# ViennaRNA/RNAcode

Measured on AMD Instinct MI355X. Metric: alignment-columns x samples scored /sec, higher is better.
Workload: dtype f32; 1 GPU; synthetic MAF 10000 blocks x 120 cols x 6 seqs, n=1000 (BASELINE configs[2]/[3]); exchange=none, fit_exp_mode=fused

## Files before the change

rnacode_amd/csrc/rc_context.cpp:

```cpp
#include <cstddef>

#include "rc_runtime.h"

extern "C" {

const char *rc_last_error(void) { return g_err.c_str(); }

void rc_default_params(rc_params *p) {
  p->Delta = -10.0f; p->Omega = -4.0f; p->omega = -2.0f;
  p->stopPenalty_0 = -9999.0f; p->stopPenalty_k = -8.0f;
  p->blosum = 62; p->sampleN = 100; p->cutoff = 1.0f; p->stopEarly = 0; p->seed_base = 42;
  std::memset(p->genetic_code, 0, sizeof p->genetic_code);
}

}

void want_hw_queues() { (void)setenv("GPU_MAX_HW_QUEUES", "8", 0); }

int table_set(rc_ctx *c, const rc_params &par, const TableSet **out) {
  char code[64];
  const char *why = nullptr;
  if (!parse_genetic_code(par.genetic_code, code, &why)) return fail(RC_ERR_ARG, why);
  if (par.blosum != 62 && par.blosum != 90) return fail(RC_ERR_ARG, "blosum must be 62 or 90");
  std::lock_guard<std::mutex> lk(c->setMutex);
  for (const auto &t : c->sets)
    if (t->blosum == par.blosum && std::memcmp(t->code, code, 64) == 0) { *out = t.get(); return RC_OK; }
  auto t = std::make_unique<TableSet>(code, par.blosum);
  t->pt.build(t->ct);
  const size_t oPair = 0, oBlosum = al256(4096), oInfo = oBlosum + al256(400 * sizeof(int)), oPep = oInfo + al256(64 * sizeof(CodeInfo)),
               oOff = oPep + al256(64 * sizeof(int)), oAb = oOff + al256(6 * sizeof(int)), total = oAb + al256(4096 * sizeof(uint16_t));
  std::vector<uint8_t> h(total, 0);
  std::memcpy(h.data() + oPair, t->pt.pair, 4096);
  int *bl = reinterpret_cast<int *>(h.data() + oBlosum);
  for (int p = 0; p < 20; p++) for (int q = 0; q < 20; q++) bl[20 * p + q] = t->ct.blosum[p][q];
  std::memcpy(h.data() + oInfo, t->pt.info, 64 * sizeof(CodeInfo));
  int *pep = reinterpret_cast<int *>(h.data() + oPep);
  for (int i = 0; i < 64; i++) pep[i] = t->ct.pep[i];
  int *off = reinterpret_cast<int *>(h.data() + oOff);
  uint16_t *ab = reinterpret_cast<uint16_t *>(h.data() + oAb);
  int n = 0;
  off[0] = 0;
  for (int a = 0; a < 64; a++) for (int b = 0; b < 64; b++) if (pep[a] == -1 || pep[b] == -1) ab[n++] = static_cast<uint16_t>(a << 6 | b);
  for (int hq = 0; hq < 4; hq++) {
    off[1 + hq] = n;
    for (int a = 0; a < 64; a++) for (int b = 0; b < 64; b++) {
      if (pep[a] == -1 || pep[b] == -1) continue;
      const int x = a ^ b;
      if (((x & 48) != 0) + ((x & 12) != 0) + ((x & 3) != 0) == hq) ab[n++] = static_cast<uint16_t>(a << 6 | b);
    }
  }
  off[5] = n;
  t->d.retired = c->retired.get();
  HIP_TRY(hipSetDevice(c->device));
  HIP_TRY(t->d.ensure(total));
  HIP_TRY(hipMemcpy(t->d.p, h.data(), total, hipMemcpyHostToDevice));
  const uint8_t *d = t->d.as<uint8_t>();
  const CodeTables standard(par.blosum);
  t->ptrs = TablePtrs{d + oPair, reinterpret_cast<const int *>(d + oPep), reinterpret_cast<const int *>(d + oBlosum),
                      reinterpret_cast<const CodeInfo *>(d + oInfo), reinterpret_cast<const int *>(d + oOff),
                      reinterpret_cast<const uint16_t *>(d + oAb), std::memcmp(standard.pep, t->ct.pep, sizeof standard.pep) == 0};
  *out = t.get();
  c->sets.push_back(std::move(t));
  return RC_OK;
}

extern "C" {

int rc_device_count(void) {
  want_hw_queues();
  int n = 0;
  if (hipGetDeviceCount(&n) != hipSuccess) return 0;
  return n;
}

int rc_host_cpus(void) { return effective_cpus(); }

void rc_ctx_trim(rc_ctx *c) {
  if (!c) return;
  (void)hipSetDevice(c->device);
  (void)hipDeviceSynchronize();
  c->retired->drain();
  c->bufPool->drain(false);
}

void rc_ctx_destroy(rc_ctx *c) {
  if (!c) return;
  (void)hipSetDevice(c->device);
  (void)hipDeviceSynchronize();
  c->retired->ctxGone.store(true);
  c->retired->drain();
  g_retired.drain();
  c->bufPool->drain(true);
  c->pool.reset();
  if (kProfiling && c->d_cellStats.p) {
    unsigned long long st[6] = {0, 0, 0, 0, 0, 0};
    if (hipMemcpy(st, c->d_cellStats.p, sizeof st, hipMemcpyDeviceToHost) == hipSuccess && st[0])
      std::fprintf(stderr, "[rc cell stats] wavefront-cells %llu, with no positive lane %llu (%.4f %%), positive lane-cells %.2f %%\n", st[0], st[1],
                   100.0 * st[1] / st[0], 100.0 * st[2] / (64.0 * st[0])),
      std::fprintf(stderr, "[rc cell stats] before the row's first event %.1f %%, event codons %.1f %%, after its last event %.1f %%, between events %.1f %%\n",
                   100.0 * st[3] / st[0], 100.0 * st[4] / st[0], 100.0 * st[5] / st[0], 100.0 * (st[0] - st[3] - st[4] - st[5]) / st[0]);
  }
  if (c->d_U) (void)hipFree(c->d_U);
  for (hipStream_t st : c->compute) if (st) (void)hipStreamDestroy(st);
  if (c->native) (void)hipStreamDestroy(c->native);
  if (c->copy) (void)hipStreamDestroy(c->copy);
  if (c->aux) (void)hipStreamDestroy(c->aux);
  if (c->tree) (void)hipStreamDestroy(c->tree);
  if (c->tree2) (void)hipStreamDestroy(c->tree2);
  for (hipStream_t st : c->classStreams) (void)hipStreamDestroy(st);
  delete c;
}

int rc_ctx_create(int device, rc_ctx **out) {
  if (!out) return fail(RC_ERR_ARG, "null out pointer");
  *out = nullptr;
  want_hw_queues();
  int n = 0;
  trace("ctx: start", nullptr);
  if (hipGetDeviceCount(&n) != hipSuccess || n <= 0)
    return fail(RC_ERR_DEVICE, "no HIP device available: the scoring path has no CPU fallback");
  trace("ctx: runtime up", nullptr);
  if (device < 0 || device >= n) return fail(RC_ERR_ARG, "device index out of range");
  HIP_TRY(hipSetDevice(device));
  std::unique_ptr<rc_ctx, void (*)(rc_ctx *)> guard(new rc_ctx(), rc_ctx_destroy);
  rc_ctx *c = guard.get();
  c->device = device;
  hipDeviceProp_t prop;
  HIP_TRY(hipGetDeviceProperties(&prop, device));
  c->numCU = prop.multiProcessorCount;
  c->totalMem = prop.totalGlobalMem;
  c->retiredCapBytes = prop.totalGlobalMem / 16;
  c->bufPool->devCap = prop.totalGlobalMem / 16;
  c->bufPool->device = device;
  static const int hostExp = exp_mode_of_host();
  c->expMode = hostExp;
  if (const char *e = std::getenv("RC_FIT_EXP")) {
    const std::string v(e);
    if (v == "generic" || v == "1") c->expMode = 1;
    else if (v == "fused" || v == "fma" || v == "2") c->expMode = 2;
    else if (v == "device" || v == "0") c->expMode = 0;
    else return fail(RC_ERR_ARG, "RC_FIT_EXP must be generic, fused or device");
  }
  for (DevBuf *d : {&c->treeJobs, &c->treeIn, &c->treeWork, &c->treeRes, &c->d_cellStats}) d->retired = c->retired.get();
  for (PinBuf *h : {&c->treeInPin, &c->treeResPin}) h->retired = c->retired.get();
  c->genericScratchWords = std::max<size_t>(static_cast<size_t>(1) << 30, prop.totalGlobalMem / 12 / sizeof(uint32_t));
  c->togetherWords = std::max<size_t>(static_cast<size_t>(1) << 30, prop.totalGlobalMem / 36 / sizeof(uint32_t));
  if (const char *e = std::getenv("RC_TOGETHER_MAX_MB")) c->togetherWords = static_cast<size_t>(std::max(0ll, std::atoll(e))) * (1u << 20) / sizeof(uint32_t);
  if (const char *e = std::getenv("RC_CLASS_STREAMS")) c->classStreamCount = std::max(1, std::min(16, std::atoi(e)));
  if (const char *e = std::getenv("RC_GRID_CAP_PER_CU")) c->gridCapPerCU = std::max(0, std::atoi(e));
  if (const char *e = std::getenv("RC_SPLIT_FACTOR")) c->splitFactor = std::max(0.0, std::atof(e));
  if (const char *e = std::getenv("RC_NATIVE_WAVES_PER_CU")) c->nativeWavesPerCU = std::max(1, std::min(32, std::atoi(e)));
  if (const char *e = std::getenv("RC_TAIL_SHARING")) c->tailSharing = std::atoi(e) != 0;
  if (const char *e = std::getenv("RC_ROW_SPLIT")) c->rowSplit = std::atoi(e) != 0;
  if (const char *e = std::getenv("RC_HIGH_OCCUPANCY")) c->highOccupancy = std::max(0, std::min(2, std::atoi(e)));
  if (prop.maxSharedMemoryPerMultiProcessor > 0) c->ldsPerCU = prop.maxSharedMemoryPerMultiProcessor;
  if (const char *e = std::getenv("RC_FAT_STREAM_MIN_ITEMS")) c->fatStreamMinItems = std::max(0ll, std::atoll(e));
  if (const char *e = std::getenv("RC_GENERIC_SCRATCH_MB")) c->genericScratchWords = std::max<size_t>(1, static_cast<size_t>(std::atoll(e))) * (1u << 20) / sizeof(uint32_t);
  int prioLow = 0, prioHigh = 0;
  HIP_TRY(hipDeviceGetStreamPriorityRange(&prioLow, &prioHigh));
  c->prioLow = prioLow; c->prioHigh = 0; c->classPrio = prioLow;
  trace("ctx: streams", nullptr);
  c->serialNative = std::getenv("RC_SERIAL_NATIVE") ? 1 : 0;
  c->stopTwoRoundsMinItems = 4LL * c->numCU * 16;
  if (const char *e = std::getenv("RC_STOP_MIN_ITEMS")) c->stopTwoRoundsMinItems = std::atoll(e);
  if (const char *e = std::getenv("RC_GENERIC_MIN_ROWS")) c->rule.genericMinRows = std::max(3, std::min(kTemplRows + 1, std::atoi(e)));
  if (const char *e = std::getenv("RC_TILED_MAX_L")) c->rule.tiledMaxL = std::max(0, std::atoi(e));
  if (const char *e = std::getenv("RC_TILED_MIN_ROWS")) c->rule.tiledMinRows = std::max(kTiledMaxKT + 2, std::min(kTemplRows + 1, std::atoi(e)));
  if (const char *e = std::getenv("RC_TILED_MAX_ROWS")) c->rule.tiledMaxRows = std::max(kTemplRows, std::min(kMaxRows, std::atoi(e)));
  if (const char *e = std::getenv("RC_TILED_WIDE_MAX_L")) c->rule.tiledWideMaxL = std::max(0, std::atoi(e));
  if (const char *e = std::getenv("RC_TILED_ANY_L_MIN_ROWS")) c->rule.tiledAnyLMinRows = std::max(kTemplRows + 1, std::atoi(e));
  if (const char *e = std::getenv("RC_STOP_ROUNDS")) c->stopRounds = std::max(2, std::min(kMaxRounds, std::atoi(e)));
  {
    rc_params std{};
    std.blosum = 62;
    const TableSet *unused = nullptr;
    RC_TRY(table_set(c, std, &unused));
    std.blosum = 90;
    RC_TRY(table_set(c, std, &unused));
  }
  trace("ctx: tables", nullptr);
  c->tieThr = float_threshold_lt(0.0001);
  if (const char *e = std::getenv("RC_LDS_MAX_BYTES")) { c->ldsMaxBytes = c->ldsMaxBytesOneRow = static_cast<size_t>(std::atol(e)); c->stageManyRows = true; }
#ifdef RC_PROFILING
  if (const char *e = std::getenv("RC_DEBUG_SKIP")) c->debugSkip = std::atoi(e);
  if (std::getenv("RC_CELL_STATS")) {
    HIP_TRY(c->d_cellStats.ensure(6 * sizeof(unsigned long long)));
    HIP_TRY(hipMemset(c->d_cellStats.p, 0, 6 * sizeof(unsigned long long)));
  }
#endif
  c->hostThreads = std::min(effective_cpus(), 32);
  if (const char *e = std::getenv("RC_HOST_THREADS")) c->hostThreads = std::max(1, std::atoi(e));
  *out = guard.release();
  return RC_OK;
}

int rc_genetic_code(int32_t ncbi_id, char out[65]) {
  if (!out) return fail(RC_ERR_ARG, "null out pointer");
  const char *aas = ncbi_code(ncbi_id);
  if (!aas) return fail(RC_ERR_ARG, "unknown genetic code id " + std::to_string(ncbi_id) +
                                    " (built in: 1-6, 9-14, 16, 21-26, 29, 30, 33; 27, 28, 31 and 32 are not supported)");
  std::memcpy(out, aas, 64);
  out[64] = '\0';
  return RC_OK;
}

int rc_ctx_set_host_threads(rc_ctx *c, int32_t threads) {
  if (!c || threads < 1) return fail(RC_ERR_ARG, "bad argument");
  if (c->inflight.load() != 0) return fail(RC_ERR_ARG, "batches are in flight");
  c->hostThreads = threads;
  c->pool.reset();
  return RC_OK;
}

int rc_ctx_host_threads(const rc_ctx *c) { return c ? c->hostThreads : 0; }

int rc_ctx_fit_exp_mode(const rc_ctx *c) { return c ? c->expMode : RC_ERR_ARG; }

}

#undef rc_default_params
#undef rc_batch_create
#undef rc_stream_create
static constexpr size_t kParamsV1Bytes = offsetof(rc_params, genetic_code);
static_assert(kParamsV1Bytes == 40, "the members of the older rc_params layout");
static rc_params params_v1(const rc_params *old) {
  rc_params p;
  std::memset(&p, 0, sizeof p);
  std::memcpy(&p, old, kParamsV1Bytes);
  return p;
}

extern "C" {

void rc_default_params(rc_params *p) {
  rc_params q;
  rc_default_params_v2(&q);
  std::memcpy(p, &q, kParamsV1Bytes);
}

int rc_batch_create(rc_ctx *ctx, const rc_block *blocks, int32_t n_blocks, const rc_params *par, rc_batch **out) {
  if (!par) return rc_batch_create_v2(ctx, blocks, n_blocks, par, out);
  const rc_params p = params_v1(par);
  return rc_batch_create_v2(ctx, blocks, n_blocks, &p, out);
}

int rc_stream_create(rc_ctx *ctx, const rc_params *par, int32_t depth, rc_stream **out) {
  if (!par) return rc_stream_create_v2(ctx, par, depth, out);
  const rc_params p = params_v1(par);
  return rc_stream_create_v2(ctx, &p, depth, out);
}

}
```

rnacode_amd/csrc/rc_launch.h:

```cpp
#pragma once
#include <hip/hip_runtime.h>

#include <cstddef>
#include <cstdint>
#include <string>

#include "rc_device.h"

namespace rc {

#ifdef RC_PROFILING
constexpr bool kProfiling = true;
#else
constexpr bool kProfiling = false;
#endif

struct NullArgs {
  const uint8_t *blob;
  const DevBlock *dblocks;
  const int *classBlocks;
  int nClassBlocks;
  const int *nBlocksPtr;
  const uint32_t *flags;
  uint32_t skipMask;
  uint32_t onlyMask;
  int tiledKT;
  int gLo, gHi;
  int sampleN;
  int Spad;
  const uint32_t *U;
  const uint8_t *pair;
  uint32_t *scratch;
  size_t scratchStride;
  float *maxima;
  unsigned long long *clampCount;
  float tieThr;
  int comboSplit;
  unsigned int *workCounter;
  unsigned int *steal;
  uint8_t *codesAll;
  size_t codesStride;
  int cacheSites;
  int reserved[3];
  int stealWait;
  int simParts, simGrid;
  unsigned int *simCounter;
  int rowParts;
  float *sbuf;
  size_t sbufStride;
  int debugSkip;
  unsigned long long *cellStats;
};

struct NativeArgs {
  uint8_t *blob;
  const DevBlock *dblocks;
  const int *blocks;
  const uint8_t *pair;
  float *tile;
  size_t tileStride;
  int nItems;
  float *fullS;
  float *sAll;
  int sAllSites;
  DevHss *hss;
  int *hssCount;
  int hssCap;
  float tieThr;
  const uint32_t *flags;
};

struct PrepArgs {
  uint8_t *blob;
  const DevBlock *dblocks;
  const int *blocks;
  int nBlocks;
  const int *modelPrefix;
  int nModels;
  const int *pep;
  bool standardCode;
  const int *prepOff;
  const uint16_t *prepAb;
  const int *blosum;
  const CodeInfo *codeInfo;
  uint32_t *flags;
  int *exactList;
  int *exactCount;
  int classOff[kClassSlots];
  ClassRule rule;
};

struct FitOut {
  double mu, lambda;
  int rc;
  int better;
};

struct FitArgs {
// ... 178 lines not shown
```

rnacode_amd/csrc/rc_null_kernel.h:

```cpp
#pragma once
#include <hip/hip_runtime.h>

#include <type_traits>
#include <utility>

#include "rc_device.h"
#include "rc_launch.h"
#include "rc_sim_core.h"

namespace rc {


template <bool SEM> __device__ __forceinline__ float ref_max(float x, float y) {
  if constexpr (SEM) return x > y ? x : y;
  else return fmaxf(x, y);
}
template <bool SEM> __device__ __forceinline__ float ref_max3(float x, float y, float z) { return ref_max<SEM>(ref_max<SEM>(x, y), z); }

template <bool SEM = false>
__device__ __forceinline__ void pair_step(int zc, float sig, float Delta, float Omega, float omega,
                                          float &s0, float &s1, float &s2) {
  if (zc == 0) {
    s0 = s0 + sig;
    s1 = s1 + omega;
// ... 423 lines not shown
            static_for<QB>([&](auto xc) {
              constexpr int x = decltype(xc)::value;
              wait_draws(ubq[x], std::integral_constant<int, SPI * (QB - 1 - x)>{});
              if (q0 + x < nnodes) node_step(q0 + x, ubq[x], [] {});
            });
          }
        } else {
          for (int q = 0; q < nnodes; q++) {
            uint32_t u[SPI];
            if constexpr (!kLean) {
#pragma unroll
              for (int t = 0; t < SPI; t++) u[t] = Ustream[ubase[t] + q * qstride];
              node_step_plain(q, u);
              continue;
            }
            fetch_draws(u, ub[0], ub[1], ub[2], ub[3]);
#pragma unroll
            for (int t = 0; t < SPI; t++) ub[t] += qstrideB;
            node_step(q, u, [&] { wait_draws(u, std::integral_constant<int, 0>{}); });
          }
        }
#pragma unroll
        for (int t = 0; t < SPI; t++) {
          const int i = i0 + t;
          if (i <= L) {
#pragma unroll
            for (int r = 0; r < N; r++) {
              const uint32_t tip = get_state(ns[t], static_cast<int>((qtipw[r >> 2] >> (8 * (r & 3))) & 255u));
              win[r] = sim_window(win[r], tip);
              if constexpr (kRevWindow) winR[r] = sim_window_rev(winR[r], tip);
            }
            if (i >= 3 && (!SIM || (i >= iLo && i <= iHi))) {
              const int ip = L + 3 - i;
              const uint32_t aF = win[0] & 63u;
              uint32_t aR = kRevWindow ? sim_rev_codon(winR[0]) : sim_ref_rev(aF);
              asm("" : "+v"(aR));
              uint8_t *siteF = reinterpret_cast<uint8_t *>(cod + static_cast<size_t>(0 * L1 + i) * PSW);
              uint8_t *siteR = reinterpret_cast<uint8_t *>(cod + static_cast<size_t>(1 * L1 + ip) * PSW);
#pragma unroll
              for (int w = 0; w < NCW; w++) {
                uint32_t wf = 0, wr = 0;
                const uint32_t mF = maskw[(0 * L1 + i) * NCW + w], mR = maskw[(1 * L1 + ip) * NCW + w];
#pragma unroll
                for (int c = 0; c < CPW; c++) {
                  const int k = w * CPW + c;
                  if (k < NK) {
                    wf |= sim_pack(pairLut[sim_index_fwd(aF, win[k + 1], sim_mask_field(mF, c))], c);
                    if constexpr (kRevWindow) wr |= sim_pack(pairLut[sim_index_rev_window(aR, winR[k + 1], sim_mask_field(mR, c))], c);
                    else wr |= sim_pack(pairLut[sim_index_rev(aR, win[k + 1], sim_mask_field(mR, c))], c);
                  }
                }
                if (w < NCW - 1) {
                  store_words(std::integral_constant<int, 4>{}, laneWord, wf, wr, siteF + w * kWave * 4, siteR + w * kWave * 4);
                } else {
                  store_words(std::integral_constant<int, LB>{}, laneTailB, wf, wr, siteF + (NCW - 1) * kWave * 4, siteR + (NCW - 1) * kWave * 4);
                }
              }
            }
          }
        }
      }
      if (clamped && (kLean ? lane == 0 : sidx < A.sampleN) && (SIM || onlyCombo <= 0)) atomicAdd(A.clampCount, static_cast<unsigned long long>(clamped));
    }
    if constexpr (SIM) continue;
    if (!helping && shared) {
      const size_t G = gridDim.x;
      if (lane == 0) {
        __hip_atomic_store(A.steal + kStealHdr + G + 2 * blockIdx.x, static_cast<unsigned int>(bi), __ATOMIC_RELAXED, __HIP_MEMORY_SCOPE_AGENT);
        __hip_atomic_store(A.steal + kStealHdr + G + 2 * blockIdx.x + 1, static_cast<unsigned int>(grp), __ATOMIC_RELAXED, __HIP_MEMORY_SCOPE_AGENT);
      }
      __builtin_amdgcn_fence(__ATOMIC_RELEASE, "agent");
      __builtin_amdgcn_s_waitcnt(0);
      if (lane == 0) {
        atomicExch(A.steal + kStealHdr + blockIdx.x, 1u);
        const unsigned int idx = atomicAdd(A.steal, 1u);
        __hip_atomic_store(A.steal + kStealHdr + 3 * G + idx, (blockIdx.x + 1u) | (static_cast<unsigned int>(home) << 24), __ATOMIC_RELAXED, __HIP_MEMORY_SCOPE_AGENT);
        atomicSub(A.steal + 1, 1u);
      }
      firstCombo = claim_part(slot);
    }

    float best = -1.0f;
    unsigned long long statCells = 0, statNoPos = 0, statPosLanes = 0, statPristine = 0, statEvent = 0, statTail = 0;
    float omega_v, Delta_v = 0.0f;
    asm volatile("v_mov_b32 %0, %1" : "=v"(omega_v) : "s"(omega));
    float rcpNk_v = 0.0f, negNk_v = 0.0f;
    if constexpr (!EXACT && (NK & (NK - 1)) != 0) {
      asm volatile("v_mov_b32 %0, %1" : "=v"(rcpNk_v) : "s"(1.0f / static_cast<float>(NK)));
      asm volatile("v_mov_b32 %0, %1" : "=v"(negNk_v) : "s"(-static_cast<float>(NK)));
    }
    if constexpr (EXACT) asm volatile("v_mov_b32 %0, %1" : "=v"(Delta_v) : "s"(Delta));
    if (!kProfiling || !(A.debugSkip & 1)) {
      Regs R;
      int curS = -1;
      for (int c = onlyCombo >= 0 ? onlyCombo : firstCombo; c < 6; c = onlyCombo >= 0 ? 6 : (shared ? claim_part(slot) : c + 1)) {
        const int s = c >= 3 ? 1 : 0, f = c - 3 * s;
        if (s != curS) {
          static_for<NK>([&](auto kc) {
            constexpr int k = decltype(kc)::value;
            R.template at<k>().lut = __float_as_int(lut[(s * NK + k) * kLutSize + lane]);
            if constexpr (kTableLookups) lds_codes[k * kWave + lane] = static_cast<uint32_t>(R.template at<k>().lut);
          });
          curS = s;
        }
        const int sites = (L - f) / 3;
        if (sites <= 0) continue;
        const uint32_t *__restrict__ sbase = cod + static_cast<size_t>(s * L1 + 3 + f) * PSW;
        constexpr int kSiteWords = 3 * PSW;
        auto word_at = [&](int j, int x) -> uint32_t {
          const uint32_t *p = sbase + static_cast<size_t>(j) * kSiteWords;
          if (x < NCW - 1) return p[x * kWave + lane];
          return static_cast<uint32_t>(reinterpret_cast<const TailT *>(p + (NCW - 1) * kWave)[lane]);
        };
        const unsigned long long *__restrict__ zbase = zw + static_cast<size_t>(s * L1 + 3 + f) * ZW;
        const unsigned long long *__restrict__ zany = zmask + static_cast<size_t>(s * 3 + f) * zmWords;
        int jc = sites;
        constexpr int kCacheSiteBytes = PSW * 4;
        if constexpr (LDSC) {
          for (int idx = 0; idx < sites * NCW; idx++) lds_codes[idx * kWave + lane] = word_at(idx / NCW, idx % NCW);
          __builtin_amdgcn_s_waitcnt(0);
        } else if constexpr (!EXACT) {
          jc = sites - (A.cacheSites < sites ? A.cacheSites : sites);
          for (int j = jc; j < sites; j++) {
            uint32_t *dst = lds_codes + kTableWords + (j - jc) * PSW;
#pragma unroll
            for (int x = 0; x < NCW - 1; x++) dst[x * kWave + lane] = word_at(j, x);
            reinterpret_cast<TailT *>(dst + (NCW - 1) * kWave)[lane] = static_cast<TailT>(word_at(j, NCW - 1));
          }
          __builtin_amdgcn_s_waitcnt(0);
        }
        const uint32_t ldsBase = static_cast<uint32_t>(reinterpret_cast<uintptr_t>(lds_codes + kTableWords));
        const uint32_t ldsLane = ldsBase + static_cast<uint32_t>(lane) * 4u;
        const uint32_t ldsTail = ldsBase + (NCW - 1) * kWave * 4u + static_cast<uint32_t>(lane) * LB;
        const uint32_t laneOff = static_cast<uint32_t>(lane) * 4u, laneTail = static_cast<uint32_t>(lane) * LB;
        [[maybe_unused]] const uint8_t *ldsBytesAll = reinterpret_cast<const uint8_t *>(lds_codes + kTableWords) - ldsBase;
        auto fetch_staged = [&](uint32_t (&w)[NCW], int j) {
          const uint32_t at = ldsLane + static_cast<uint32_t>(j) * (NCW * kWave * 4u);
#pragma unroll
          for (int x = 0; x < NCW; x++) {
#ifdef RC_PLAIN_FETCH
            w[x] = *reinterpret_cast<const uint32_t *>(ldsBytesAll + at + x * kWave * 4);
#else
            asm volatile("ds_read_b32 %0, %1 offset:%2" : "=v"(w[x]) : "v"(at), "n"(x * kWave * 4));
#endif
          }
        };
        auto fetch_staged_at = [&](uint32_t (&w)[NCW], auto site) {
          constexpr int off = staged_off(decltype(site){});
          static_assert(off + NCW * kWave * 4 <= 65536, "ds_read offset: 16 bits");
          const uint32_t at = site.at;
#pragma unroll
          for (int x = 0; x < NCW; x++) {
#ifdef RC_PLAIN_FETCH
            w[x] = *reinterpret_cast<const uint32_t *>(ldsBytesAll + at + off + x * kWave * 4);
#else
            asm volatile("ds_read_b32 %0, %1 offset:%2" : "=v"(w[x]) : "v"(at), "n"(off + x * kWave * 4));
#endif
          }
        };
        auto fetch_cached = [&](uint32_t (&w)[NCW], int j) {
          const uint32_t off = static_cast<uint32_t>(j - jc) * kCacheSiteBytes;
#ifdef RC_PLAIN_FETCH
          if constexpr (NCW > 1) {
#pragma unroll
            for (int x = 0; x < NCW - 1; x++) w[x] = *reinterpret_cast<const uint32_t *>(ldsBytesAll + ldsLane + off + x * kWave * 4);
          }
          w[NCW - 1] = static_cast<uint32_t>(*reinterpret_cast<const TailT *>(ldsBytesAll + ldsTail + off));
#else
          if constexpr (NCW > 1) {
            const uint32_t at = ldsLane + off;
#pragma unroll
            for (int x = 0; x < NCW - 1; x++) asm volatile("ds_read_b32 %0, %1 offset:%2" : "=v"(w[x]) : "v"(at), "n"(x * kWave * 4));
          }
          const uint32_t att = ldsTail + off;
          if constexpr (LB == 1) asm volatile("ds_read_u8 %0, %1" : "=v"(w[NCW - 1]) : "v"(att));
          else if constexpr (LB == 2) asm volatile("ds_read_u16 %0, %1" : "=v"(w[NCW - 1]) : "v"(att));
          else asm volatile("ds_read_b32 %0, %1" : "=v"(w[NCW - 1]) : "v"(att));
#endif
        };
        auto fetch_global = [&](uint32_t (&w)[NCW], const uint32_t *p) {
          const uint32_t lo = laneOff + 0u, lt = laneTail + 0u;
#ifdef RC_PLAIN_FETCH
          const uint8_t *pb = reinterpret_cast<const uint8_t *>(p);
#pragma unroll
          for (int x = 0; x < NCW - 1; x++) w[x] = *reinterpret_cast<const uint32_t *>(pb + lo + x * kWave * 4);
          w[NCW - 1] = static_cast<uint32_t>(*reinterpret_cast<const TailT *>(pb + lt + (NCW - 1) * kWave * 4));
          return;
#endif
#pragma unroll
// ... 198 lines not shown
            wvB = wvB + omega_v;
            float sumA = 0.0f, sumB = 0.0f;
            static_for<NK>([&](auto kc) {
              constexpr int k = decltype(kc)::value;
              auto &ra = R.template at<k>();
              auto &rb = RB.template at<k>();
              ra.s0 = ra.s0 + sig[k];
              const float ma = fmaxf(ra.s0, wvA);
              sumA = (k == 0) ? ma : sumA + ma;
              rb.s0 = rb.s0 + sig[k];
              const float mb = fmaxf(rb.s0, wvB);
              sumB = (k == 0) ? mb : sumB + mb;
            });
            vB = finish(sumB);
            return finish(sumA);
          };
          auto fast2 = [&](uint32_t (&w)[NCW], auto jn, float &vB, auto kd) -> float {
            float sig[NK];
            lookup(w, sig, jn, std::false_type{}, kd);
            float sumA = 0.0f, sumB = 0.0f;
            static_for<NK>([&](auto kc) {
              constexpr int k = decltype(kc)::value;
              auto &ra = R.template at<k>();
              auto &rb = RB.template at<k>();
              ra.s0 = ra.s0 + sig[k];
              ra.s1 = ra.s1 + omega_v;
              ra.s2 = ra.s2 + omega_v;
              const float ma = fmaxf(fmaxf(ra.s0, ra.s1), ra.s2);
              sumA = (k == 0) ? ma : sumA + ma;
              rb.s0 = rb.s0 + sig[k];
              rb.s1 = rb.s1 + omega_v;
              rb.s2 = rb.s2 + omega_v;
              const float mb = fmaxf(fmaxf(rb.s0, rb.s1), rb.s2);
              sumB = (k == 0) ? mb : sumB + mb;
            });
            vB = finish(sumB);
            return finish(sumA);
          };
          auto tail2 = [&](uint32_t (&w)[NCW], auto jn, float &vB, auto kd) -> float {
            float sig[NK];
            lookup(w, sig, jn, std::false_type{}, kd);
            float sumA = 0.0f, sumB = 0.0f;
            static_for<NK>([&](auto kc) {
              constexpr int k = decltype(kc)::value;
              auto &ra = R.template at<k>();
              auto &rb = RB.template at<k>();
              ra.s0 = ra.s0 + sig[k];
              ra.s1 = ra.s1 + omega_v;
              const float ma = fmaxf(ra.s0, ra.s1);
              sumA = (k == 0) ? ma : sumA + ma;
              rb.s0 = rb.s0 + sig[k];
              rb.s1 = rb.s1 + omega_v;
              const float mb = fmaxf(rb.s0, rb.s1);
              sumB = (k == 0) ? mb : sumB + mb;
            });
            vB = finish(sumB);
            return finish(sumA);
          };
          auto event2 = [&](uint32_t (&w)[NCW], int j, int jn, float &vB) -> float {
            float sig[NK];
            lookup(w, sig, jn, std::true_type{}, std::true_type{});
            unsigned long long z[ZW];
#pragma unroll
            for (int x = 0; x < ZW; x++) z[x] = zbase[static_cast<size_t>(3 * j) * ZW + x];
            float sumA = 0.0f, sumB = 0.0f;
            static_for<NK>([&](auto kc) {
              constexpr int k = decltype(kc)::value;
              auto &ra = R.template at<k>();
              auto &rb = RB.template at<k>();
              const int zc = static_cast<int>((z[k >> 5] >> (2 * (k & 31))) & 3ull);
              pair_step(zc, sig[k], Delta, Omega, omega, ra.s0, ra.s1, ra.s2);
              const float ma = fmaxf(fmaxf(ra.s0, ra.s1), ra.s2);
              sumA = (k == 0) ? ma : sumA + ma;
              pair_step(zc, sig[k], Delta, Omega, omega, rb.s0, rb.s1, rb.s2);
              const float mb = fmaxf(fmaxf(rb.s0, rb.s1), rb.s2);
              sumB = (k == 0) ? mb : sumB + mb;
            });
            vB = finish(sumB);
            return finish(sumA);
          };
          int a = 0;
          int pendRow = -1, pendExtra = 0, pendN = 0;
          while (a < sites || pendRow >= 0) {
            if (pendRow < 0 && a + 2 < sites && !((zany[a >> 6] >> (a & 63)) & 1ull)) {
              sample_scan_row_begin(st, best, static_cast<uint32_t>(a));
              static_for<NK>([&](auto kc) {
                constexpr int k = decltype(kc)::value;
                auto &r = R.template at<k>();
                r.s0 = r.s1 = r.s2 = 0.0f;
                auto &rb = RB.template at<k>();
                rb.s0 = rb.s1 = rb.s2 = 0.0f;
              });
              uint32_t wcur[NCW];
              load_words(a, wcur);
              int j = a;
              float j2f = static_cast<float>(2 * a + 1);
              float wvA = 0.0f, wvB = 0.0f;
              asm volatile("v_mov_b32 %0, 0" : "=v"(wvA));
              asm volatile("v_mov_b32 %0, 0" : "=v"(wvB));
              {
                const float v = pristine_cell(wcur, wvA, a + 1, std::true_type{});
                sample_scan_step(st, v, j2f, negTie);
                asm volatile("v_add_f32 %0, %1, %0" : "+v"(j2f) : "v"(two_v));
                j = a + 1;
              }
              const int extra = (sites - 1 - a > kBuf) ? sites - 1 - a - kBuf : 0;
              const int b0 = a + 1 + extra;
              auto keep = [&](float vB, int jj) {
                const int idx = jj > b0 ? jj - b0 : 0;
                buf[idx] = vB;
              };
              auto pair_cell = [&](uint32_t (&w)[NCW], int jj, int jn, auto kd, auto &&fn) {
                float vB;
                const float v = fn(w, jn, vB, kd);
                sample_scan_step(st, v, j2f, negTie);
                keep(vB, jj);
                const float two_c = two_v;
                asm volatile("v_add_f32 %0, %1, %0" : "+v"(j2f) : "v"(two_c));
              };
              auto dspan = [&](int e, auto &&fn) {
                if constexpr (!LDSC && !EXACT && MODE == 0)
                  deep_pairs(j, wcur, e, [&](uint32_t (&w)[NCW], int jj, int jn) { pair_cell(w, jj, jn, DeepFetch{}, fn); });
                if constexpr (LDSC) {
                  for (const int pe = e < b0 ? e : b0; j < pe; j++) {
                    float vB;
                    const float v = fn(wcur, j + 1, vB, std::true_type{});
                    sample_scan_step(st, v, j2f, negTie);
                    const float two_c = two_v;
                    asm volatile("v_add_f32 %0, %1, %0" : "+v"(j2f) : "v"(two_c));
                  }
                  const int ge = e < sites - 1 ? e : sites - 1;
                  for (; j + kGroup <= ge; j += kGroup) {
                    const uint32_t at = ldsLane + static_cast<uint32_t>(j + 1) * (NCW * kWave * 4u);
                    float vB[kGroup];
                    static_for<kGroup>([&](auto uc) {
                      constexpr int u = decltype(uc)::value;
                      const float v = fn(wcur, StagedSite<u * NCW * kWave * 4>{at}, vB[u], std::true_type{});
                      sample_scan_step(st, v, j2f, negTie);
                      const float two_c = two_v;
                      asm volatile("v_add_f32 %0, %1, %0" : "+v"(j2f) : "v"(two_c));
                    });
                    int idxRaw = j - b0;
                    asm volatile("" : "+s"(idxRaw));
                    const int idx = idxRaw & (kBuf - 1);
                    __builtin_amdgcn_sched_barrier(0);
                    static_for<kGroup>([&](auto uc) {
                      constexpr int u = decltype(uc)::value;
                      buf[idx + u] = vB[u];
                    });
                    __builtin_amdgcn_sched_barrier(0);
                  }
                }
                for (; j < e; j++) pair_cell(wcur, j, j + 1 < sites ? j + 1 : j, std::true_type{}, fn);
              };
              {
                dspan(next_event(j, sites), [&](uint32_t (&w)[NCW], auto jn, float &vB, auto kd) { return pristine2(w, wvA, wvB, jn, vB, kd); });
                static_for<NK>([&](auto kc) {
                  constexpr int k = decltype(kc)::value;
                  auto &r = R.template at<k>();
                  r.s1 = r.s2 = wvA;
                  auto &rb = RB.template at<k>();
                  rb.s1 = rb.s2 = wvB;
                });
              }
              while (j < sites) {
                if ((zany[j >> 6] >> (j & 63)) & 1ull) {
                  const int jev = j;
                  pair_cell(wcur, j, j + 1 < sites ? j + 1 : j, std::true_type{}, [&](uint32_t (&w)[NCW], int jn, float &vB, auto) { return event2(w, jev, jn, vB); });
                  j++;
                }
                const int e = next_event(j, sites);
                if (e == sites) {
                  static_for<NK>([&](auto kc) {
                    constexpr int k = decltype(kc)::value;
                    auto &r = R.template at<k>();
                    r.s1 = fmaxf(r.s1, r.s2);
                    auto &rb = RB.template at<k>();
                    rb.s1 = fmaxf(rb.s1, rb.s2);
                  });
                  dspan(e, [&](uint32_t (&w)[NCW], auto jn, float &vB, auto kd) { return tail2(w, jn, vB, kd); });
                }
                dspan(e, [&](uint32_t (&w)[NCW], auto jn, float &vB, auto kd) { return fast2(w, jn, vB, kd); });
              }
#pragma unroll
              for (int x = 0; x < NCW; x++) asm volatile("s_waitcnt lgkmcnt(0)" : "+v"(wcur[x]));
              sample_scan_row_end(st, static_cast<uint32_t>(a));
              pendRow = a + 1; pendExtra = extra; pendN = sites - b0;
              a += 2;
            } else {
              const bool pend = pendRow >= 0;
              const int row = pend ? pendRow : a;
              const int jend = pend ? row + pendExtra : ((row == sites - 1) ? sites - 1 : sites);
              float j2f = static_cast<float>(2 * row + 1);
              sample_scan_row_begin(st, best, static_cast<uint32_t>(row));
              static_for<NK>([&](auto kc) {
                constexpr int k = decltype(kc)::value;
                auto &r = R.template at<k>();
                r.s0 = r.s1 = r.s2 = 0.0f;
              });
              uint32_t wcur[NCW];
              load_words(row, wcur);
              int j = row;
              auto take = [&](float v) {
                sample_scan_step(st, v, j2f, negTie);
                asm volatile("v_add_f32 %0, %1, %0" : "+v"(j2f) : "v"(two_v));
              };
              auto one = [&](auto &&cell) {
                const int jn = j + 1 < sites ? j + 1 : j;
                take(cell(wcur, jn, std::true_type{}));
              };
              {
                const int e = next_event(j, jend);
                float wv = 0.0f;
                asm volatile("v_mov_b32 %0, 0" : "=v"(wv));
                for (; j < e; j++) one([&](uint32_t (&w)[NCW], int jn, auto kd) {
                  if constexpr (kProfiling) statPristine++;
                  return pristine_cell(w, wv, jn, kd);
                });
                static_for<NK>([&](auto kc) {
                  constexpr int k = decltype(kc)::value;
                  auto &r = R.template at<k>();
                  r.s1 = r.s2 = wv;
                });
              }
              while (j < jend) {
                if ((zany[j >> 6] >> (j & 63)) & 1ull) {
                  if constexpr (kProfiling) statEvent++;
                  const int jj = j;
                  one([&](uint32_t (&w)[NCW], int jn, auto kd) { return event_cell(w, jj, jn, kd, std::false_type{}); });
                  j++;
                }
                const int e = next_event(j, jend);
                if (e == jend) {
                  static_for<NK>([&](auto kc) {
                    constexpr int k = decltype(kc)::value;
                    auto &r = R.template at<k>();
                    r.s1 = fmaxf(r.s1, r.s2);
                  });
                  for (; j < e; j++) one([&](uint32_t (&w)[NCW], int jn, auto kd) {
                    if constexpr (kProfiling) statTail++;
                    return tail_cell(w, jn, kd);
                  });
                }
                for (; j < e; j++) one([&](uint32_t (&w)[NCW], int jn, auto kd) { return fast_cell(w, jn, kd); });
              }
#pragma unroll
              for (int x = 0; x < NCW; x++) {
                if constexpr (LDSC) asm volatile("s_waitcnt lgkmcnt(0)" : "+v"(wcur[x]));
                else asm volatile("s_waitcnt vmcnt(0) lgkmcnt(0)" : "+v"(wcur[x]));
              }
              if (pend) {
                [&]() {
#pragma unroll
                  for (int idx = 0; idx < kBuf; idx++) {
                    if (idx >= pendN) return;
                    sample_scan_step(st, buf[idx], j2f, negTie);
                    asm volatile("v_add_f32 %0, %1, %0" : "+v"(j2f) : "v"(two_v));
                  }
                }();
                pendRow = -1;
              } else {
                a += 1;
              }
              sample_scan_row_end(st, static_cast<uint32_t>(row));
            }
          }
        } else {
          int aLo = 0, aHi = sites;
          float *sdst = nullptr;
          if constexpr (ROWS) {
            const long long total = static_cast<long long>(sites) * (sites + 1) / 2;
            auto row_at = [&](long long cellsBefore) {
              int a = 0;
              long long cum = 0;
              while (a < sites && cum < cellsBefore) { cum += sites - a; a++; }
              return a;
            };
// ... 15 lines not shown
            int j = a;
            float j2f = static_cast<float>(2 * a + 1);
            auto take = [&](float v) {
              if constexpr (ROWS) { *sdst = v; sdst += kWave; }
              else {
                sample_scan_step(st, v, j2f, negTie);
                asm volatile("v_add_f32 %0, %1, %0" : "+v"(j2f) : "v"(two_v));
              }
            };
            auto one = [&](auto &&cell) {
              const int jn = j + 1 < sites ? j + 1 : j;
              uint32_t wnext[NCW];
              if constexpr (EXACT) load_words(jn, wnext);
              take(cell(wcur, jn, std::true_type{}));
              if constexpr (EXACT) {
#pragma unroll
                for (int x = 0; x < NCW; x++) wcur[x] = wnext[x];
              }
            };
            auto span = [&](int e, auto &&cell) {
              if constexpr (kDeep) deep_pairs(j, wcur, e, [&](uint32_t (&w)[NCW], int, int jn) { take(cell(w, jn, DeepFetch{})); });
              for (; j < e; j++) one(cell);
            };
            if constexpr (EXACT) {
              if (nanSem)
                for (; j < jend; j++) {
                  const int jj = j;
                  one([&](uint32_t (&w)[NCW], int jn, auto kd) { return event_cell(w, jj, jn, kd, std::true_type{}); });
                }
            }
            {
              const int e = next_event(j, jend);
              float wv = 0.0f;
              asm volatile("v_mov_b32 %0, 0" : "=v"(wv));
              span(e, [&](uint32_t (&w)[NCW], int jn, auto kd) {
                if constexpr (kProfiling) statPristine++;
                return pristine_cell(w, wv, jn, kd);
              });
              static_for<NK>([&](auto kc) {
                constexpr int k = decltype(kc)::value;
                auto &r = R.template at<k>();
                r.s1 = r.s2 = wv;
              });
            }
            while (j < jend) {
              if ((zany[j >> 6] >> (j & 63)) & 1ull) {
                if constexpr (kProfiling) statEvent++;
                const int jj = j;
                one([&](uint32_t (&w)[NCW], int jn, auto kd) { return event_cell(w, jj, jn, kd, std::false_type{}); });
                j++;
              }
              const int e = next_event(j, jend);
              if (e == jend) {
                static_for<NK>([&](auto kc) {
                  constexpr int k = decltype(kc)::value;
                  auto &r = R.template at<k>();
                  r.s1 = fmaxf(r.s1, r.s2);
                });
                span(e, [&](uint32_t (&w)[NCW], int jn, auto kd) {
                  if constexpr (kProfiling) statTail++;
                  return tail_cell(w, jn, kd);
                });
              }
              span(e, [&](uint32_t (&w)[NCW], int jn, auto kd) { return fast_cell(w, jn, kd); });
            }
            if constexpr (!EXACT) {
#pragma unroll
              for (int x = 0; x < NCW; x++) {
                if constexpr (LDSC) asm volatile("s_waitcnt lgkmcnt(0)" : "+v"(wcur[x]));
                else asm volatile("s_waitcnt vmcnt(0) lgkmcnt(0)" : "+v"(wcur[x]));
              }
            }
            if constexpr (ROWS) { if (a == sites - 1) sdst += kWave; }
            else sample_scan_row_end(st, static_cast<uint32_t>(a));
          }
        }
        if constexpr (!ROWS) sample_scan_last(st, best);
      }
    }
    if constexpr (kProfiling) {
      if (A.cellStats && lane == 0) {
        atomicAdd(A.cellStats, statCells); atomicAdd(A.cellStats + 1, statNoPos); atomicAdd(A.cellStats + 2, statPosLanes);
        atomicAdd(A.cellStats + 3, statPristine); atomicAdd(A.cellStats + 4, statEvent); atomicAdd(A.cellStats + 5, statTail);
      }
    }
    if (!ROWS && sidx < A.sampleN) {
      float *dst = maxima + static_cast<size_t>(db->out_index) * A.sampleN + sidx;
      if (A.comboSplit || shared) { if (best > -1.0f) atomicMax(reinterpret_cast<int *>(dst), __float_as_int(best)); }
      else *dst = best;
    }
  }
}

constexpr int null_min_waves(int NK, bool EXACT, bool DUAL, int MODE) { return DUAL ? 4 : (EXACT || MODE != 0) ? 1 : NK == 6 ? 6 : (NK == 9 || NK == 10) ? 5 : (NK >= 16 && NK <= 21) ? 4 : (NK >= 24 && NK <= 29) ? 3 : 1; }
template <int NK, bool LDSC, bool EXACT, bool DUAL = false, int MODE = 0>
__global__ __launch_bounds__(64) __attribute__((amdgpu_waves_per_eu(null_min_waves(NK, EXACT, DUAL, MODE))))
void k_null(NullArgs A, const uint8_t *__restrict__ blob,
                                             const DevBlock *__restrict__ dblocks, const int *__restrict__ classBlocks,
                                             const uint32_t *__restrict__ flags, const uint32_t *__restrict__ Ustream, const uint8_t *__restrict__ pairTab,
                                             uint32_t *__restrict__ scratch, float *__restrict__ maxima) {
  null_body<NK, LDSC, EXACT, DUAL, MODE>(A, blob, dblocks, classBlocks, flags, Ustream, pairTab, scratch, maxima);
}

constexpr int hi_occ_waves(int NK) { return (NK >= 6 && NK <= 8) ? 6 : (NK >= 10 && NK <= 12) ? 5 : 0; }
template <int NK>
__global__ __launch_bounds__(64) __attribute__((amdgpu_waves_per_eu(hi_occ_waves(NK) ? hi_occ_waves(NK) : 1)))
void k_null_occ(NullArgs A, const uint8_t *__restrict__ blob, const DevBlock *__restrict__ dblocks, const int *__restrict__ classBlocks,
                const uint32_t *__restrict__ flags, const uint32_t *__restrict__ Ustream, const uint8_t *__restrict__ pairTab,
                uint32_t *__restrict__ scratch, float *__restrict__ maxima) {
  null_body<NK, false, false, false>(A, blob, dblocks, classBlocks, flags, Ustream, pairTab, scratch, maxima);
}


template <int NK>
inline int null_occupancy_one(NullKind kind, size_t lds) {
  int nb = 0;
  hipError_t e = hipErrorInvalidValue;
  switch (kind) {
    case NullKind::Exact: e = hipOccupancyMaxActiveBlocksPerMultiprocessor(&nb, k_null<NK, false, true>, 64, lds); break;
    case NullKind::Staged: if constexpr (NK < kFastRows) e = hipOccupancyMaxActiveBlocksPerMultiprocessor(&nb, k_null<NK, true, false>, 64, lds); break;
    case NullKind::StagedTwoRow: if constexpr (NK <= kDualRowsMaxNK) e = hipOccupancyMaxActiveBlocksPerMultiprocessor(&nb, k_null<NK, true, false, true>, 64, lds); break;
    case NullKind::L2: if constexpr (NK < kFastRows) e = hipOccupancyMaxActiveBlocksPerMultiprocessor(&nb, k_null<NK, false, false>, 64, lds); break;
    case NullKind::L2Occ: if constexpr (hi_occ_waves(NK) != 0) e = hipOccupancyMaxActiveBlocksPerMultiprocessor(&nb, k_null_occ<NK>, 64, lds); break;
    case NullKind::L2TwoRow: if constexpr (NK >= 3 && NK <= kDualRowsMaxNK) e = hipOccupancyMaxActiveBlocksPerMultiprocessor(&nb, k_null<NK, false, false, true>, 64, lds); break;
    case NullKind::RowSplit: if constexpr (NK < kFastRows) e = hipOccupancyMaxActiveBlocksPerMultiprocessor(&nb, k_null<NK, false, false, false, 1>, 64, lds); break;
    default: break;
  }
  return e == hipSuccess ? nb : 0;
}

#define RC_NULL_GO(...) hipLaunchKernelGGL((__VA_ARGS__), dim3(grid), dim3(64), lds, stream, a, a.blob, a.dblocks, a.classBlocks, a.flags, a.U, a.pair, a.scratch, a.maxima)
template <int NK>
inline bool launch_null_one(NullKind kind, const NullArgs &a, int grid, size_t lds, hipStream_t stream) {
  switch (kind) {
    case NullKind::Exact: RC_NULL_GO(k_null<NK, false, true>); return true;
    case NullKind::Staged:
      if constexpr (NK < kFastRows) {
        if (lds > 48 * 1024)
          (void)hipFuncSetAttribute(reinterpret_cast<const void *>(k_null<NK, true, false>), hipFuncAttributeMaxDynamicSharedMemorySize, static_cast<int>(lds));
        RC_NULL_GO(k_null<NK, true, false>);
        return true;
      }
      break;
    case NullKind::StagedTwoRow: if constexpr (NK <= kDualRowsMaxNK) { RC_NULL_GO(k_null<NK, true, false, true>); return true; } break;
    case NullKind::L2: if constexpr (NK < kFastRows) { RC_NULL_GO(k_null<NK, false, false>); return true; } break;
    case NullKind::L2Occ: if constexpr (hi_occ_waves(NK) != 0) { RC_NULL_GO(k_null_occ<NK>); return true; } break;
    case NullKind::L2TwoRow: if constexpr (NK >= 3 && NK <= kDualRowsMaxNK) { RC_NULL_GO(k_null<NK, false, false, true>); return true; } break;
    case NullKind::RowSplit:
      if constexpr (NK < kFastRows) {
        hipLaunchKernelGGL((k_null<NK, false, false, false, 2>), dim3(a.simGrid), dim3(64), kPhaseALds, stream, a, a.blob, a.dblocks,
                           a.classBlocks, a.flags, a.U, a.pair, a.scratch, a.maxima);
        RC_NULL_GO(k_null<NK, false, false, false, 1>);
        return true;
      }
      break;
    default: break;
  }
  return false;
}
#undef RC_NULL_GO

#define RC_DEFINE_NULL_RANGE(SUFFIX, LO, HI)                                                                                    \
  template <int NK> static int occ_rec_##SUFFIX(int nk, NullKind k, size_t lds) {                                                \
    if constexpr (NK > HI) return 0;                                                                                             \
    else return nk == NK ? null_occupancy_one<NK>(k, lds) : occ_rec_##SUFFIX<NK + 1>(nk, k, lds);                                 \
  }                                                                                                                              \
// ... 11 lines not shown
```

Measured before the change: 28.59 billion alignment-columns*samples/s.

## Let two-row walk start on event rows and add a two-cell group tail

The two-row walk now also runs when row a begins on an event codon. It skips the pristine first cell and resets row a+1's accumulators after the event pair, so such rows no longer fall back to single-row processing. The staged LDS loop gains a group-of-two tail, so fewer cells go through the one-at-a-time path. Profiling counters for these paths are added but compile only under RC_PROFILING. The extra branches on ev0 add control flow and may raise register pressure in the hot loop.

```diff
diff --git a/rnacode_amd/csrc/rc_context.cpp b/rnacode_amd/csrc/rc_context.cpp
--- a/rnacode_amd/csrc/rc_context.cpp
+++ b/rnacode_amd/csrc/rc_context.cpp
@@ -93,12 +93,18 @@
   c->bufPool->drain(true);
   c->pool.reset();
   if (kProfiling && c->d_cellStats.p) {
-    unsigned long long st[6] = {0, 0, 0, 0, 0, 0};
+    unsigned long long st[kCellStatSlots] = {};
     if (hipMemcpy(st, c->d_cellStats.p, sizeof st, hipMemcpyDeviceToHost) == hipSuccess && st[0])
       std::fprintf(stderr, "[rc cell stats] wavefront-cells %llu, with no positive lane %llu (%.4f %%), positive lane-cells %.2f %%\n", st[0], st[1],
                    100.0 * st[1] / st[0], 100.0 * st[2] / (64.0 * st[0])),
       std::fprintf(stderr, "[rc cell stats] before the row's first event %.1f %%, event codons %.1f %%, after its last event %.1f %%, between events %.1f %%\n",
                    100.0 * st[3] / st[0], 100.0 * st[4] / st[0], 100.0 * st[5] / st[0], 100.0 * (st[0] - st[3] - st[4] - st[5]) / st[0]);
+    if (st[13]) {
+      const double items = st[13] / 6.0;
+      std::fprintf(stderr, "[rc two-row walk] per item: cell pairs in groups of four %.2f, in groups of two %.2f, one at a time %.2f (event pairs %.2f), "
+                   "rows alone %.2f, their cells %.2f, cells of rows a + 1 made again %.2f\n", st[6] / items, st[7] / items, st[8] / items, st[12] / items,
+                   st[11] / items, st[9] / items, st[10] / items);
+    }
   }
   if (c->d_U) (void)hipFree(c->d_U);
   for (hipStream_t st : c->compute) if (st) (void)hipStreamDestroy(st);
@@ -184,8 +190,8 @@
 #ifdef RC_PROFILING
   if (const char *e = std::getenv("RC_DEBUG_SKIP")) c->debugSkip = std::atoi(e);
   if (std::getenv("RC_CELL_STATS")) {
-    HIP_TRY(c->d_cellStats.ensure(6 * sizeof(unsigned long long)));
-    HIP_TRY(hipMemset(c->d_cellStats.p, 0, 6 * sizeof(unsigned long long)));
+    HIP_TRY(c->d_cellStats.ensure(kCellStatSlots * sizeof(unsigned long long)));
+    HIP_TRY(hipMemset(c->d_cellStats.p, 0, kCellStatSlots * sizeof(unsigned long long)));
   }
 #endif
   c->hostThreads = std::min(effective_cpus(), 32);
diff --git a/rnacode_amd/csrc/rc_launch.h b/rnacode_amd/csrc/rc_launch.h
--- a/rnacode_amd/csrc/rc_launch.h
+++ b/rnacode_amd/csrc/rc_launch.h
@@ -14,6 +14,7 @@
 #else
 constexpr bool kProfiling = false;
 #endif
+constexpr int kCellStatSlots = 14;
 
 struct NullArgs {
   const uint8_t *blob;
diff --git a/rnacode_amd/csrc/rc_null_kernel.h b/rnacode_amd/csrc/rc_null_kernel.h
--- a/rnacode_amd/csrc/rc_null_kernel.h
+++ b/rnacode_amd/csrc/rc_null_kernel.h
@@ -529,6 +529,7 @@
 
     float best = -1.0f;
     unsigned long long statCells = 0, statNoPos = 0, statPosLanes = 0, statPristine = 0, statEvent = 0, statTail = 0;
+    unsigned long long statG4 = 0, statG2 = 0, statOne = 0, statEvPair = 0, statAloneCells = 0, statPendCells = 0, statAloneRows = 0, statParts = 0;
     float omega_v, Delta_v = 0.0f;
     asm volatile("v_mov_b32 %0, %1" : "=v"(omega_v) : "s"(omega));
     float rcpNk_v = 0.0f, negNk_v = 0.0f;
@@ -552,6 +553,7 @@
         }
         const int sites = (L - f) / 3;
         if (sites <= 0) continue;
+        if constexpr (kProfiling) statParts++;
         const uint32_t *__restrict__ sbase = cod + static_cast<size_t>(s * L1 + 3 + f) * PSW;
         constexpr int kSiteWords = 3 * PSW;
         auto word_at = [&](int j, int x) -> uint32_t {
@@ -916,28 +918,32 @@
           int a = 0;
           int pendRow = -1, pendExtra = 0, pendN = 0;
           while (a < sites || pendRow >= 0) {
-            if (pendRow < 0 && a + 2 < sites && !((zany[a >> 6] >> (a & 63)) & 1ull)) {
+            if (pendRow < 0 && a + 2 < sites) {
+              const bool ev0 = (zany[a >> 6] >> (a & 63)) & 1ull;
               sample_scan_row_begin(st, best, static_cast<uint32_t>(a));
               static_for<NK>([&](auto kc) {
                 constexpr int k = decltype(kc)::value;
                 auto &r = R.template at<k>();
                 r.s0 = r.s1 = r.s2 = 0.0f;
-                auto &rb = RB.template at<k>();
-                rb.s0 = rb.s1 = rb.s2 = 0.0f;
               });
               uint32_t wcur[NCW];
               load_words(a, wcur);
               int j = a;
               float j2f = static_cast<float>(2 * a + 1);
               float wvA = 0.0f, wvB = 0.0f;
-              asm volatile("v_mov_b32 %0, 0" : "=v"(wvA));
-              asm volatile("v_mov_b32 %0, 0" : "=v"(wvB));
-              {
+              if (!ev0) {
+                asm volatile("v_mov_b32 %0, 0" : "=v"(wvA));
                 const float v = pristine_cell(wcur, wvA, a + 1, std::true_type{});
                 sample_scan_step(st, v, j2f, negTie);
                 asm volatile("v_add_f32 %0, %1, %0" : "+v"(j2f) : "v"(two_v));
                 j = a + 1;
               }
+              static_for<NK>([&](auto kc) {
+                constexpr int k = decltype(kc)::value;
+                auto &rb = RB.template at<k>();
+                rb.s0 = rb.s1 = rb.s2 = 0.0f;
+              });
+              if (!ev0) asm volatile("v_mov_b32 %0, 0" : "=v"(wvB));
               const int extra = (sites - 1 - a > kBuf) ? sites - 1 - a - kBuf : 0;
               const int b0 = a + 1 + extra;
               auto keep = [&](float vB, int jj) {
@@ -957,6 +963,7 @@
                   deep_pairs(j, wcur, e, [&](uint32_t (&w)[NCW], int jj, int jn) { pair_cell(w, jj, jn, DeepFetch{}, fn); });
                 if constexpr (LDSC) {
                   for (const int pe = e < b0 ? e : b0; j < pe; j++) {
+                    if constexpr (kProfiling) statOne++;
                     float vB;
                     const float v = fn(wcur, j + 1, vB, std::true_type{});
                     sample_scan_step(st, v, j2f, negTie);
@@ -964,10 +971,12 @@
                     asm volatile("v_add_f32 %0, %1, %0" : "+v"(j2f) : "v"(two_c));
                   }
                   const int ge = e < sites - 1 ? e : sites - 1;
-                  for (; j + kGroup <= ge; j += kGroup) {
+                  auto group = [&](auto gc) {
+                    constexpr int G = decltype(gc)::value;
+                    if constexpr (kProfiling) { if (G == kGroup) statG4 += G; else statG2 += G; }
                     const uint32_t at = ldsLane + static_cast<uint32_t>(j + 1) * (NCW * kWave * 4u);
-                    float vB[kGroup];
-                    static_for<kGroup>([&](auto uc) {
+                    float vB[G];
+                    static_for<G>([&](auto uc) {
                       constexpr int u = decltype(uc)::value;
                       const float v = fn(wcur, StagedSite<u * NCW * kWave * 4>{at}, vB[u], std::true_type{});
                       sample_scan_step(st, v, j2f, negTie);
@@ -978,16 +987,21 @@
                     asm volatile("" : "+s"(idxRaw));
                     const int idx = idxRaw & (kBuf - 1);
                     __builtin_amdgcn_sched_barrier(0);
-                    static_for<kGroup>([&](auto uc) {
+                    static_for<G>([&](auto uc) {
                       constexpr int u = decltype(uc)::value;
                       buf[idx + u] = vB[u];
                     });
                     __builtin_amdgcn_sched_barrier(0);
-                  }
+                  };
+                  for (; j + kGroup <= ge; j += kGroup) group(std::integral_constant<int, kGroup>{});
+                  if (j + 2 <= ge) { group(std::integral_constant<int, 2>{}); j += 2; }
                 }
-                for (; j < e; j++) pair_cell(wcur, j, j + 1 < sites ? j + 1 : j, std::true_type{}, fn);
+                for (; j < e; j++) {
+                  if constexpr (kProfiling) statOne++;
+                  pair_cell(wcur, j, j + 1 < sites ? j + 1 : j, std::true_type{}, fn);
+                }
               };
-              {
+              if (!ev0) {
                 dspan(next_event(j, sites), [&](uint32_t (&w)[NCW], auto jn, float &vB, auto kd) { return pristine2(w, wvA, wvB, jn, vB, kd); });
                 static_for<NK>([&](auto kc) {
                   constexpr int k = decltype(kc)::value;
@@ -1000,8 +1014,16 @@
               while (j < sites) {
                 if ((zany[j >> 6] >> (j & 63)) & 1ull) {
                   const int jev = j;
+                  if constexpr (kProfiling) { statOne++; statEvPair++; }
                   pair_cell(wcur, j, j + 1 < sites ? j + 1 : j, std::true_type{}, [&](uint32_t (&w)[NCW], int jn, float &vB, auto) { return event2(w, jev, jn, vB); });
                   j++;
+                  if (jev == a) {
+                    static_for<NK>([&](auto kc) {
+                      constexpr int k = decltype(kc)::value;
+                      auto &rb = RB.template at<k>();
+                      rb.s0 = rb.s1 = rb.s2 = 0.0f;
+                    });
+                  }
                 }
                 const int e = next_event(j, sites);
                 if (e == sites) {
@@ -1027,6 +1049,10 @@
               const int jend = pend ? row + pendExtra : ((row == sites - 1) ? sites - 1 : sites);
               float j2f = static_cast<float>(2 * row + 1);
               sample_scan_row_begin(st, best, static_cast<uint32_t>(row));
+              if constexpr (kProfiling) {
+                if (pend) statPendCells += jend - row;
+                else { statAloneRows++; statAloneCells += jend - row; }
+              }
               static_for<NK>([&](auto kc) {
                 constexpr int k = decltype(kc)::value;
                 auto &r = R.template at<k>();
@@ -1208,6 +1234,8 @@
       if (A.cellStats && lane == 0) {
         atomicAdd(A.cellStats, statCells); atomicAdd(A.cellStats + 1, statNoPos); atomicAdd(A.cellStats + 2, statPosLanes);
         atomicAdd(A.cellStats + 3, statPristine); atomicAdd(A.cellStats + 4, statEvent); atomicAdd(A.cellStats + 5, statTail);
+        atomicAdd(A.cellStats + 6, statG4); atomicAdd(A.cellStats + 7, statG2); atomicAdd(A.cellStats + 8, statOne); atomicAdd(A.cellStats + 9, statAloneCells);
+        atomicAdd(A.cellStats + 10, statPendCells); atomicAdd(A.cellStats + 11, statAloneRows); atomicAdd(A.cellStats + 12, statEvPair); atomicAdd(A.cellStats + 13, statParts);
       }
     }
     if (!ROWS && sidx < A.sampleN) {
```

Result: no change. 28.61 billion alignment-columns*samples/s, median of 4 (+0.1%).
